# Yelp/nrtsearch

Hardware: AMD Instinct MI355X
Metric: queries/sec, 10M-doc 5-term BM25 top-1000 (higher is better)
Workload: dtype f32

## Files before the change

include/nrtgpu_dev.h:

```cpp
#ifndef NRTGPU_DEV_H
#define NRTGPU_DEV_H
#include "nrtgpu.h"
#ifdef __cplusplus
extern "C" {
#endif
int  nrtgpu_bench_closed_loop(nrtgpu_ctx* ctx, const nrtgpu_seg* const* segs, const int32_t* doc_bases, int32_t n_segs,
                              const nrtgpu_bm25_query* queries, int32_t n_queries, int32_t clients, int32_t duration_ms,
                              double* out4);
int  nrtgpu_debug_hold_coalescers(nrtgpu_ctx* ctx, int32_t hold);
int  nrtgpu_debug_coalescer_pending(nrtgpu_ctx* ctx, int32_t which);
int  nrtgpu_debug_dist_inject(nrtgpu_ctx* ctx, int32_t step, int32_t failed_query);
int64_t nrtgpu_debug_live_segments(nrtgpu_ctx* ctx);
int  nrtgpu_debug_spec_counters(nrtgpu_ctx* ctx, int64_t* out3);
int  nrtgpu_debug_term_lookup(const nrtgpu_seg* seg, int32_t field_id, int64_t term_hash, int32_t* kind, int32_t* shift, int64_t* bytes);
int  nrtgpu_debug_knn_bounds(int32_t sim, int32_t dim, double q_norm2, double q_l1, float q_absmax, double nv_max, double nv_min,
                             float rows_absmax, float score_boost, double m, double s, double* out10);

#define NRTGPU_FLAG_PROFILE (7 << 8)
int  nrtgpu_get_scan_profile(nrtgpu_ctx* ctx, double* out16);
int  nrtgpu_get_maxscore_profile(nrtgpu_ctx* ctx, double* out16);
int64_t nrtgpu_get_maxscore_item_walls(nrtgpu_ctx* ctx, uint64_t* out, int64_t cap_slots, int64_t* n_items);

#ifdef __cplusplus
}
#endif
#endif
```

nrtsearch_amd/_lib.py:

```python
from __future__ import annotations

import ctypes as C
import os

_HERE = os.path.dirname(os.path.abspath(__file__))
LIB_PATH = os.environ.get("NRTGPU_LIB_PATH") or os.path.join(_HERE, "libnrtgpu.so")

NRTGPU_OK = 0
NRTGPU_ERR_INVALID_ARG = -1
NRTGPU_ERR_HIP = -2
NRTGPU_ERR_OOM = -3
NRTGPU_ERR_UNSUPPORTED = -4
NRTGPU_ERR_STATE = -5
NRTGPU_ERR_TIMEOUT = -6
NRTGPU_MAX_K = 1024
NRTGPU_MAX_TERMS = 32
NRTGPU_TILE_DOCS = 1024
NRTGPU_FLAG_NO_PREFETCH = 1
NRTGPU_FLAG_NO_FIXED_POINT = 2
NRTGPU_FLAG_NO_MASK_VARIANT = 4
NRTGPU_FLAG_NO_LIVE_FOLD = 8
NRTGPU_FLAG_NO_PRUNE = 16
NRTGPU_FLAG_PACKED_POSTINGS = 32
NRTGPU_FLAG_BLOCKING_WAIT = 64
# ... 11 lines not shown
    "nrtgpu_search_bm25_coalesced", "nrtgpu_set_coalescing", "nrtgpu_query_supported",
    "nrtgpu_merge_topk_device", "nrtgpu_knn_exact", "nrtgpu_knn_exact_coalesced", "nrtgpu_knn_search", "nrtgpu_rescore_vectors", "nrtgpu_search_hybrid_batch",
    "nrtgpu_int_to_byte4", "nrtgpu_byte4_to_int", "nrtgpu_bm25_idf", "nrtgpu_bm25_avgdl",
    "nrtgpu_bm25_norm_cache", "nrtgpu_slices", "nrtgpu_plan_item_counts", "nrtgpu_fixed_point_scale", "nrtgpu_get_stats", "nrtgpu_reset_stats",
    "nrtgpu_set_slicing",
    "nrtgpu_blend", "nrtgpu_dist_unique_id", "nrtgpu_dist_init", "nrtgpu_dist_search_bm25_batch", "nrtgpu_dist_allgather_merge", "nrtgpu_segment_fork",
    "nrtgpu_search_bm25_batch_device_begin", "nrtgpu_pending_wait", "nrtgpu_set_thread_deadline_ns", "nrtgpu_monotonic_ns", "nrtgpu_last_diagnostics", "nrtgpu_dist_close", "nrtgpu_dist_owned_range", "nrtgpu_dist_search_bm25_batch_mode", "nrtgpu_dist_exchange_merge", "nrtgpu_dist_exchange_merge_checked", "nrtgpu_search_bm25_shard_device_begin", "nrtgpu_note_shard_speculation", "nrtgpu_dist_knn_exact", "nrtgpu_dist_search_hybrid_batch",
    "nrtgpu_knn_exact_relation", "nrtgpu_set_speculation", "nrtgpu_set_shard_share", "nrtgpu_set_thread_slices",
    "nrtgpu_segment_add_byte_vectors", "nrtgpu_knn_exact_bytes", "nrtgpu_knn_search_bytes", "nrtgpu_byte_vector_score",
    "nrtgpu_rescore_byte_vectors", "nrtgpu_search_hybrid_bytes_batch",
]
DEV_SYMBOLS = [
    "nrtgpu_bench_closed_loop", "nrtgpu_debug_hold_coalescers", "nrtgpu_debug_coalescer_pending", "nrtgpu_debug_live_segments",
    "nrtgpu_debug_spec_counters", "nrtgpu_get_scan_profile", "nrtgpu_get_maxscore_profile", "nrtgpu_get_maxscore_item_walls",
    "nrtgpu_debug_dist_inject", "nrtgpu_debug_term_lookup", "nrtgpu_debug_knn_bounds",
]
DEV_LIB_PATH = os.path.join(_HERE, "libnrtgpu_dev.so")


class Config(C.Structure):
    _fields_ = [("device_id", C.c_int32), ("max_batch", C.c_int32), ("target_items", C.c_int32),
                ("collect_timing", C.c_int32), ("flags", C.c_int32), ("host_threads", C.c_int32),
                ("lookup_budget_pct", C.c_int32), ("reserved", C.c_int32)]


class Term(C.Structure):
    _fields_ = [("field_id", C.c_int32), ("cache_slot", C.c_int32), ("term_hash", C.c_int64),
                ("weight", C.c_float), ("occur", C.c_int32)]


# ... 125 lines not shown
    L.nrtgpu_knn_exact_relation.argtypes = [vp, vp, vp, C.c_int32, C.c_int32, C.c_int32, C.c_int32]
    L.nrtgpu_reset_stats.restype = None
    if hasattr(L, "nrtgpu_debug_hold_coalescers"):
        L.nrtgpu_debug_hold_coalescers.argtypes = [vp, C.c_int32]
        L.nrtgpu_debug_live_segments.argtypes = [vp]
        L.nrtgpu_debug_live_segments.restype = C.c_int64
        L.nrtgpu_debug_spec_counters.argtypes = [vp, vp]
        L.nrtgpu_debug_spec_counters.restype = C.c_int
        L.nrtgpu_get_maxscore_item_walls.argtypes = [vp, vp, C.c_int64, C.POINTER(C.c_int64)]
        L.nrtgpu_get_maxscore_item_walls.restype = C.c_int64
        L.nrtgpu_debug_coalescer_pending.argtypes = [vp, C.c_int32]
        L.nrtgpu_debug_dist_inject.argtypes = [vp, C.c_int32, C.c_int32]
        L.nrtgpu_get_scan_profile.argtypes = [vp, vp]
        L.nrtgpu_get_maxscore_profile.argtypes = [vp, vp]
        L.nrtgpu_debug_term_lookup.argtypes = [vp, i32, i64, C.POINTER(i32), C.POINTER(i32), C.POINTER(i64)]
    if hasattr(L, "nrtgpu_debug_knn_bounds"):
        L.nrtgpu_debug_knn_bounds.argtypes = [i32, i32, C.c_double, C.c_double, f32, C.c_double, C.c_double, f32, f32, C.c_double, C.c_double, vp]
    L.nrtgpu_set_slicing.argtypes = [vp, i32, i32, i32]
    L.nrtgpu_blend.argtypes = [i32, vp, vp, vp, vp, i32, i32, i32, i32, C.POINTER(TopDocs)]
    L.nrtgpu_dist_unique_id.argtypes = [vp]
    L.nrtgpu_dist_init.argtypes = [vp, i32, i32, vp]
    L.nrtgpu_dist_search_bm25_batch.argtypes = [vp, vp, vp, i32, C.POINTER(Bm25Query), i32, C.POINTER(TopDocs)]
    L.nrtgpu_dist_allgather_merge.argtypes = [vp, i32, i32, vp, vp, vp, vp, vp, C.POINTER(TopDocs)]
    L.nrtgpu_segment_fork.argtypes = [vp, vp, i32, C.POINTER(vp)]
    L.nrtgpu_search_bm25_batch_device_begin.argtypes = [vp, vp, vp, i32, C.POINTER(Bm25Query), i32, i32, vp, vp, vp, C.c_int64, vp]
    L.nrtgpu_pending_wait.argtypes = [vp]
    L.nrtgpu_set_thread_deadline_ns.argtypes = [C.c_int64]
    L.nrtgpu_set_thread_deadline_ns.restype = None
    L.nrtgpu_monotonic_ns.argtypes = []
    L.nrtgpu_monotonic_ns.restype = C.c_int64
# ... 19 lines not shown
```

nrtsearch_amd/api.py:

```python
from __future__ import annotations

import ctypes as C
import dataclasses
import os
import threading
from typing import Dict, List, Optional, Sequence, Tuple, Union

import numpy as np

from . import _lib
from ._lib import NrtGpuError

INT_MAX = 2**31 - 1
TOTAL_HITS_THRESHOLD = 1000


EXCHANGE_ALLGATHER, EXCHANGE_ALLTOALL = 0, 1
EXCHANGE_NO_SPECULATION = 0x100


@dataclasses.dataclass(frozen=True)
class TermQuery:
    field: int
    term: int
# ... 193 lines not shown
        out = np.zeros(16, dtype=np.float64)
        _lib.check(_lib.load().nrtgpu_get_scan_profile(self._h, out.ctypes.data))
        names = ["prologue_cycles", "rendezvous_wait_cycles", "rendezvous_cycles", "walk_cycles", "epilogue_cycles",
                 "rendezvous", "compactions", "subtiles", "rz_select_cycles", "sparse_subtiles", "rz_keep_cycles",
                 "rz_publish_append_cycles", "candidate_subtiles", "maybe_subtiles", "last_wave_finish_cycles",
                 "first_wave_finish_cycles"]
        return dict(zip(names, out.tolist()))

    def maxscore_profile(self) -> dict:
        out = np.zeros(16, dtype=np.float64)
        _lib.check(_lib.load().nrtgpu_get_maxscore_profile(self._h, out.ctypes.data))
        names = ["windows", "compactions", "chunks", "postings_streamed", "postings_surviving", "docs_evaluated", "lookups",
                 "candidates", "prologue_cycles", "item_cycles", "waves_meeting_cycles", "waves_idle_cycles", "waves_part_prologue_cycles",
                 "waves_walk_cycles", "last_wave_out_cycles", "epilogue_cycles"]
        return dict(zip(names, out.tolist()))

    @staticmethod
    def set_thread_deadline(seconds_from_now: Optional[float]) -> None:
        L = _lib.load()
        L.nrtgpu_set_thread_deadline_ns(0 if seconds_from_now is None else int(L.nrtgpu_monotonic_ns() + seconds_from_now * 1e9))

    @staticmethod
    def last_diagnostics() -> dict:
        d = _lib.Diagnostics()
        _lib.check(_lib.load().nrtgpu_last_diagnostics(C.byref(d)))
        return {n: getattr(d, n) for n, _ in _lib.Diagnostics._fields_ if n != "reserved"}

    def reset_stats(self) -> None:
        _lib.load().nrtgpu_reset_stats(self._h)

# ... 635 lines not shown
    return out, sh[:n].tolist()


def debug_knn_bounds(sim: int, dim: int, q_norm2: float, q_l1: float, q_absmax: float, nv_max: float, nv_min: float,
                     rows_absmax: float, score_boost: float = 1.0, m: float = 0.0, s: float = 0.0) -> dict:
    out = np.zeros(10, dtype=np.float64)
    _lib.check(_lib.load().nrtgpu_debug_knn_bounds(int(sim), int(dim), float(q_norm2), float(q_l1), C.c_float(q_absmax), float(nv_max),
                                                   float(nv_min), C.c_float(rows_absmax), C.c_float(score_boost), float(m), float(s),
                                                   out.ctypes.data))
    names = ("e32", "e16", "result_upper32", "result_upper16", "estimate_lower32", "estimate_lower16", "q_scale", "rows_scale")
    d = {n: float(out[i]) for i, n in enumerate(names)}
    d["q_scale_usable"], d["rows_scale_usable"] = bool(out[8]), bool(out[9])
    return d


def blend(retriever_docs: Sequence[np.ndarray], retriever_scores: Optional[Sequence[np.ndarray]] = None,
          boosts: Optional[Sequence[float]] = None, mode: str = "rrf", k: int = 60, start_hit: int = 0, top_hits: int = 10) -> TopDocs:
    n = len(retriever_docs)
    docs = [np.ascontiguousarray(d, dtype=np.int32) for d in retriever_docs]
    scs = [np.ascontiguousarray(s_, dtype=np.float32) for s_ in retriever_scores] if retriever_scores is not None else None
    dp = (C.c_void_p * max(n, 1))(*[d.ctypes.data for d in docs])
    sp = (C.c_void_p * max(n, 1))(*[s_.ctypes.data for s_ in scs]) if scs is not None else None
    counts = np.asarray([len(d) for d in docs], dtype=np.int32)
    b = np.ascontiguousarray(boosts, dtype=np.float32) if boosts is not None else None
    cap = max(int(top_hits), 1)
    od, os_ = np.zeros(cap, np.int32), np.zeros(cap, np.float32)
    out = _lib.TopDocs()
    out.capacity = cap
    out.docs = od.ctypes.data_as(C.POINTER(C.c_int32))
    out.scores = os_.ctypes.data_as(C.POINTER(C.c_float))
# ... 22 lines not shown
```

nrtsearch_amd/csrc/devtools.cpp:

```cpp
#include "runtime_internal.h"
#include "../../include/nrtgpu_dev.h"

extern "C" int nrtgpu_bench_closed_loop(nrtgpu_ctx* ctx, const nrtgpu_seg* const* segs, const int32_t* doc_bases,
                                        int32_t n_segs, const nrtgpu_bm25_query* queries, int32_t n_queries,
                                        int32_t clients, int32_t duration_ms, double* out4) {
  if (!ctx || !queries || !out4 || n_queries <= 0 || clients <= 0 || duration_ms <= 0)
    return fail(NRTGPU_ERR_INVALID_ARG, "bad closed-loop arguments");
  std::vector<std::vector<float>> lat((size_t)clients);
  std::vector<int> rcs((size_t)clients, 0);
  std::vector<std::string> errs((size_t)clients);
  const auto t_begin = std::chrono::steady_clock::now();
  const auto t_stop = t_begin + std::chrono::milliseconds(duration_ms);
  auto client = [&](int c) {
    int32_t kmax = 1;
    for (int i = 0; i < n_queries; ++i) kmax = std::max(kmax, queries[i].k);
    std::vector<int32_t> docs((size_t)kmax);
    std::vector<float> scores((size_t)kmax);
    size_t i = (size_t)c * 7919u;
    for (;;) {
      const auto t0 = std::chrono::steady_clock::now();
      if (t0 >= t_stop) break;
      nrtgpu_topdocs o{};
      o.capacity = kmax;
      o.docs = docs.data();
// ... 33 lines not shown
  const double e_rel = (double)hostmath::knn_e_rel(), b = (double)score_boost;
  const float e32 = hostmath::knn_bound32(sim, dim, q_norm2, nv_max, b);
  const float e16 = hostmath::knn_bound16(sim, dim, q_norm2, q_l1, 1.0 / (double)q_scale, nv_max, nv_min, 1.0 / (double)rows_scale, b);
  out10[0] = (double)e32;
  out10[1] = (double)e16;
  out10[2] = knn_result_upper(sim, m, (double)e32, e_rel, b);
  out10[3] = knn_result_upper(sim, m, (double)e16, e_rel, b);
  out10[4] = knn_estimate_lower(sim, s, (double)e32, e_rel, b);
  out10[5] = knn_estimate_lower(sim, s, (double)e16, e_rel, b);
  out10[6] = (double)q_scale;
  out10[7] = (double)rows_scale;
  out10[8] = q_ok ? 1.0 : 0.0;
  out10[9] = rows_ok ? 1.0 : 0.0;
  return NRTGPU_OK;
}
```

nrtsearch_amd/csrc/maxscore.hip:

```cpp
#include <hip/hip_runtime.h>
#include <stdint.h>

#include "bm25_common.hiph"

namespace nrtgpu {

constexpr int kMsWinWords = kMsWinDocs / 32;
constexpr int kSl = kMsSlots;
typedef uint32_t u32x2 __attribute__((ext_vector_type(2)));
typedef const NRT_GLOBAL u32x2* gvec2_ptr;

struct alignas(16) WClause {
  uint64_t docids, fnorm;
  uint64_t begin;
  uint32_t count, pad0;
  float    weight;
  int32_t  fx_scale;
  uint32_t flags;
  uint32_t pad;
  uint64_t u_after;
  uint64_t look;
  uint64_t cells, start;
};
static_assert(sizeof(WClause) == 80, "WClause layout");

struct MsSmem {
  uint64_t cand[kMsCandCap];
  uint32_t tab[kTabTerms][kTabEntries];
  float    cache[kLdsCaches][256];
  uint32_t seen[kMsWaves][kMsWinWords];
  WClause  wc[kMsWaves][kMsMaxTerms];
  TopkScratch sc;
  uint64_t theta;
  uint64_t thr;
  uint32_t cnt;
  uint32_t cnt_valid;
  uint32_t rz_flag;
  uint32_t wins_started;
  uint32_t spec_at;
  uint32_t q_wins;
  uint32_t spec_z16;
  uint32_t spec_grow16;
  unsigned long long* spec_slot;
  uint64_t pick;
  uint32_t role[4];
  uint32_t prune_on;
  uint32_t slot_hits[kSliceSlots];
  uint32_t slot_slice[kSliceSlots];
  uint64_t prof[16];
};
static_assert(sizeof(MsSmem) <= 160 * 1024, "the MaxScore workgroup owns one CU's 160 KiB LDS");

// ... 57 lines not shown
__device__ __forceinline__ ms_args_ptr ms_fresh(const MsArgs* p) {
  uint32_t lo = (uint32_t)(uintptr_t)p, hi = (uint32_t)((uintptr_t)p >> 32);
  asm volatile("" : "+v"(lo), "+v"(hi));
  lo = (uint32_t)__builtin_amdgcn_readfirstlane((int)lo);
  hi = (uint32_t)__builtin_amdgcn_readfirstlane((int)hi);
  return (ms_args_ptr)(((uintptr_t)hi << 32) | (uintptr_t)lo);
}

__device__ __noinline__ void ms_compact(__attribute__((address_space(3))) MsSmem* sp, uint32_t k, int fx_E,
                                        unsigned long long* theta_g, const DExchange* xch, uint32_t query) {
  MsSmem& s = *(MsSmem*)sp;
  const uint32_t tid = threadIdx.x;
  const uint32_t cnt_raw = s.cnt;
  const uint32_t cnt0 = cnt_raw > (uint32_t)kMsCandCap ? s.cnt_valid : cnt_raw;
  __syncthreads();
  const bool exchanging = xch && xch->world > 1u;
  uint32_t r = 0;
  if (s.spec_z16 != 0u && !exchanging && __hip_atomic_load(&s.prune_on, __ATOMIC_RELAXED, __HIP_MEMORY_SCOPE_WORKGROUP) != 0u) {
    const float m = (float)k * fminf(1.0f, (float)s.wins_started / (float)max(s.q_wins, 1u));
    const float rr = m + (float)s.spec_z16 * (1.0f / 16.0f) * sqrtf(m) + 2.0f;
    r = rr < (float)k ? (uint32_t)rr : 0u;
  }
  uint64_t guess = 0;
  if (cnt0 > k) {
    const uint32_t k2 = exchanging ? (k + xch->world - 2u) / (xch->world - 1u) : r;
    const uint64_t thr = topk_kth_union<kMsThreads>(s.cand, cnt0, k, &s.sc, [](auto&&) {}, k2);
    const uint32_t q2_hi = s.sc.q2_hi;
    const uint32_t kept = topk_keep_ge<kMsThreads, kMsCandCap>(s.cand, cnt0, thr, &s.sc);
    if (tid == 0) {
      s.cnt = kept;
      if (thr > s.theta) {
        s.theta = thr;
        s.thr = acc_threshold<true>(thr, fx_E);
      }
      atomicMax(theta_g, (unsigned long long)thr);
      s.prof[1] += 1;
    }
    if (!exchanging && r != 0u && q2_hi != 0u) guess = (uint64_t)q2_hi << 32;
    if (xch && tid < 64u) {
      const uint64_t pb = exchange_bound(*xch, query, q2_hi != 0u ? (uint64_t)q2_hi << 32 : 0ull, tid);
      if (tid == 0 && pb > s.theta) {
        s.theta = pb;
        s.thr = acc_threshold<true>(pb, fx_E);
// ... 13 lines not shown
    }
    const uint32_t ws = s.wins_started;
    s.spec_at = ws >= s.q_wins ? 0u : max(ws * s.spec_grow16 / 16u, ws + (uint32_t)kMsWaves);
  }
  __syncthreads();
  if (tid == 0) s.rz_flag = 0;
  __syncthreads();
}

__device__ __forceinline__ bool ms_meet(MsSmem& s, uint32_t k, int fx_E, unsigned long long* theta_g, const DExchange* xch = nullptr,
                                        uint32_t query = 0) {
  __syncthreads();
  if (!__hip_atomic_load(&s.rz_flag, __ATOMIC_RELAXED, __HIP_MEMORY_SCOPE_WORKGROUP)) return false;
  ms_compact((__attribute__((address_space(3))) MsSmem*)&s, k, fx_E, theta_g, xch, query);
  return true;
}

__device__ __forceinline__ bool ms_reserve(MsSmem& s, uint32_t lane, uint32_t mine, uint32_t& pos) {
  const uint32_t incl = scan64_dpp(mine);
  const uint32_t wave_total = (uint32_t)__builtin_amdgcn_readlane((int)incl, 63);
  uint32_t wbase = 0;
  if (lane == 0) {
    wbase = atomicAdd(&s.cnt, wave_total);
    if (wbase + wave_total > (uint32_t)kMsCandCap) {
      if (wbase <= (uint32_t)kMsCandCap) s.cnt_valid = wbase;
      __hip_atomic_store(&s.rz_flag, 1u, __ATOMIC_RELAXED, __HIP_MEMORY_SCOPE_WORKGROUP);
    }
  }
  wbase = (uint32_t)__builtin_amdgcn_readfirstlane((int)wbase);
  pos = wbase + incl - mine;
// ... 115 lines not shown
    const uint32_t mode = item.flags & 3u;
    const uint32_t win_tiles = (uint32_t)kMsWinTiles >> ((item.flags >> 2) & 3u);
    const uint32_t msm = SHAPES ? q.min_should_match : 0u;
    const bool use_max = SHAPES && q.combine_max != 0u;
    const uint32_t sec_mode = TWO ? q.sec_mode : kMsSecNone;
    const float tie_breaker = TWO ? q.tie_breaker : 0.0f;
    auto loosen = [&](uint64_t t) { return (TWO && sec_mode == kMsSecReqOpt) ? max(t - (t >> 21), (uint64_t)2) - (uint64_t)1 : t; };
    unsigned int* const my_prune_g = as_global(ap->q_prune) + item.query;
    const uint64_t after_key = q.has_after ? pack_key(q.after_score, (uint32_t)q.after_doc) : ~0ull;

    {
      const uint32_t n_lds = min(item.n_caches, (uint32_t)kLdsCaches) * 256u;
      const float* const caches = as_global(ap->caches);
      for (uint32_t i = tid; i < n_lds; i += kMsThreads) (&s.cache[0][0])[i] = caches[item.cache_off + i];
    }
    if (tid == 0) {
      const uint64_t theta0 = __hip_atomic_load(my_theta_g, __ATOMIC_RELAXED, __HIP_MEMORY_SCOPE_AGENT);
      s.theta = theta0;
      s.thr = acc_threshold<true>(theta0, fx_E);
      s.cnt = 0;
      s.cnt_valid = 0;
      s.rz_flag = 0;
      if (!helper) {
        const unsigned long long now0 = (unsigned long long)wall_clock64();
        __hip_atomic_store(hp.item_t0 + my_item, now0, __ATOMIC_RELAXED, __HIP_MEMORY_SCOPE_AGENT);
        if (my_item == 0u) __hip_atomic_store(hp.t_start, now0, __ATOMIC_RELAXED, __HIP_MEMORY_SCOPE_AGENT);
      }
      s.prune_on = mode == kMsModePrune ? 1u : 0u;
      const bool spec = hp.spec_g != nullptr && hp.spec_z16 != 0u;
      s.wins_started = 0;
      s.q_wins = spec ? as_global(ap->q_wins)[item.query] : 0u;
      s.spec_z16 = spec ? hp.spec_z16 : 0u;
      s.spec_slot = spec ? as_global(hp.spec_g) + item.query : nullptr;
      s.spec_at = spec ? max(hp.spec_sched & 255u, 1u) : 0u;
      s.spec_grow16 = max((hp.spec_sched >> 8) & 255u, 17u);
      for (int i = 0; i < kSliceSlots; ++i) s.slot_hits[i] = s.slot_slice[i] = 0u;
      for (int i = 0; i < 16; ++i) s.prof[i] = 0;
    }
    const uint64_t t_item0 = PROF ? __builtin_readcyclecounter() : 0ull;
    const uint64_t wall0 = PROF ? wall_clock64() : 0ull;
    uint64_t tc_meet = 0, tc_part = 0, tc_walk = 0;
    __syncthreads();
    if (xch && tid < 64u) {
      const uint64_t pb = exchange_bound(*xch, item.query, 0ull, tid);
      if (tid == 0 && pb > s.theta) {
        s.theta = pb;
        s.thr = acc_threshold<true>(pb, fx_E);
      }
    }
    for (uint32_t slot = 0; slot < item.n_tabs; ++slot) {
// ... 130 lines not shown
        w.start = mt.start;
        wcl[lane] = w;
      }
      const uint32_t req_mask = TWO ? (uint32_t)__builtin_amdgcn_ballot_w64(lane < n_terms && (mt.tab_slot & kTabSlotRequired) != 0u) : 0u;
      const uint32_t first_req = req_mask != 0u ? (uint32_t)__builtin_ctz(req_mask) : 0xFFu;
      if (PROF) tc_part += __builtin_readcyclecounter() - t_part0;

      for (;;) {
        const uint64_t t_win0 = PROF ? __builtin_readcyclecounter() : 0ull;
        const uint32_t ta = (part.tile_begin & ~(win_tiles - 1u)) + (g - win_base) * win_tiles;
        const uint32_t t0 = max(ta, part.tile_begin);
        const uint32_t t1 = min(ta + win_tiles, part.tile_end);
        const uint32_t doc_lo = t0 * (uint32_t)kTileDocs;
        const uint32_t doc_span = min(t1 * (uint32_t)kTileDocs, part.max_doc) - doc_lo;
        if (PROF) pc_wins += 1;
        if (lane == 0) {
          const uint32_t ws = atomicAdd(&s.wins_started, 1u) + 1u, at = s.spec_at;
          if (at != 0u && ws >= at) __hip_atomic_store(&s.rz_flag, 1u, __ATOMIC_RELAXED, __HIP_MEMORY_SCOPE_WORKGROUP);
        }
        uint32_t g_new = 0;
        if (lane == 0) g_new = (uint32_t)kMsWaves + __hip_atomic_fetch_add(win_next_g, 1u, __ATOMIC_RELAXED, __HIP_MEMORY_SCOPE_AGENT);
        uint64_t theta_other = 0, thr_other = 0;
        if (multi_item) {
          theta_other = __hip_atomic_load(my_theta_g, __ATOMIC_RELAXED, __HIP_MEMORY_SCOPE_AGENT);
          thr_other = acc_threshold<true>(theta_other, fx_E);
          if (mode == kMsModeCount && lane == 0 && __hip_atomic_load(my_prune_g, __ATOMIC_RELAXED, __HIP_MEMORY_SCOPE_AGENT) != 0u)
            __hip_atomic_store(&s.prune_on, 1u, __ATOMIC_RELAXED, __HIP_MEMORY_SCOPE_WORKGROUP);
        }
        uint32_t my_lo = 0, my_hi = 0;
        if (lane < n_terms) {
          my_lo = my_cells[t0 >> my_shift];
          my_hi = my_cells[((t1 - 1u) >> my_shift) + 1u];
        }
// ... 473 lines not shown
    if (tid == 0) {
      as_global(ape->item_counts)[out_slot] = n;
      if (helper)
        as_global(hpe.help_query)[out_slot - hpe.slot_base] = item.query + 1u;
      uint32_t hits = 0;
      for (int i = 0; i < kSliceSlots; ++i) {
        const uint32_t h = s.slot_hits[i];
        hits += h;
        if (h != 0u && q.gte_floor != 0xFFFFFFFFu) atomicAdd(as_global(ape->slice_sum) + q.slice_base + s.slot_slice[i], h);
      }
      const bool pruned = s.prune_on != 0u && (s.theta != 0ull || __hip_atomic_load(my_theta_g, __ATOMIC_RELAXED, __HIP_MEMORY_SCOPE_AGENT) != 0ull);
      as_global(ape->item_hits)[out_slot] = (uint64_t)hits + (pruned ? kHitsPrunedUnit : 0ull);
      if (PROF && ape->item_prof) {
  #ifndef NRT_MS_PHASE_CLOCKS
        s.prof[5] = hits;
  #endif
        const uint64_t t_end = __builtin_readcyclecounter();
        s.prof[9] = t_end - t_item0;
        s.prof[15] = t_end - t_epi0;
        for (int i = 0; i < 16; ++i) as_global(ape->item_prof)[(size_t)out_slot * 16 + i] = s.prof[i];
        if (hpe.walls) {
          unsigned long long* const wr = as_global(hpe.walls) + (size_t)out_slot * 8;
          wr[0] = wall0;
          wr[1] = wall_clock64();
          wr[2] = (unsigned long long)my_item | ((unsigned long long)item.flags << 32);
          wr[3] = s.prof[0];
          wr[4] = wall_entry;
          wr[5] = ((unsigned long long)((uint32_t)__builtin_amdgcn_s_getreg((31 << 11) | 20) & 15u) << 8) |
                  (unsigned long long)(((uint32_t)__builtin_amdgcn_s_getreg((31 << 11) | 4) >> 8) & 255u);
          wr[6] = (unsigned long long)round | ((unsigned long long)item.query << 32);
// ... 81 lines not shown
  const uint32_t n_cells = ((max_doc - 1u) >> shift) + 1u;
  uint32_t* const out = (uint32_t*)(look_base + t_look[t]);
  const uint32_t stride = gridDim.x * blockDim.x;
  for (uint32_t i = blockIdx.x * blockDim.x + threadIdx.x; i <= n_cells; i += stride) {
    const uint64_t bound = (uint64_t)i << shift;
    uint32_t lo = 0, hi = n;
    while (lo < hi) {
      const uint32_t mid = (lo + hi) >> 1;
      if ((uint64_t)dd[mid] < bound) lo = mid + 1u;
      else hi = mid;
    }
    out[i] = lo;
  }
}

void launch_bm25_maxscore(hipStream_t stream, bool profile, bool packed, int shapes, const MsArgs& args, const MsArgs* args_d) {
  const uint32_t n_items = args.help.n_own;
  if (n_items == 0) return;
  const uint32_t grid = args.help.persistent ? std::min(n_items + args.help.n_help, std::max(args.help.n_cus, 1u)) : n_items + args.help.n_help;
#define NRT_MS_LAUNCH(P, K, S) hipLaunchKernelGGL((bm25_maxscore_kernel<P, K, S>), dim3(grid), dim3(kMsThreads), 0, stream, args_d)
#define NRT_MS_LAUNCH_S(P, K)          \
  do {                                 \
    if (shapes == 2) NRT_MS_LAUNCH(P, K, 2);      \
    else if (shapes == 1) NRT_MS_LAUNCH(P, K, 1); \
    else NRT_MS_LAUNCH(P, K, 0);                  \
  } while (0)
#ifdef NRTGPU_DEV
  if (profile) {
    if (packed) NRT_MS_LAUNCH_S(true, true);
    else NRT_MS_LAUNCH_S(true, false);
// ... 42 lines not shown
```

nrtsearch_amd/csrc/runtime.cpp:

```cpp
#include "runtime_internal.h"

namespace nrtgpu {
namespace rt {
thread_local std::string g_last_error;
thread_local int64_t g_deadline_ns = 0;
thread_local nrtgpu_diagnostics g_diag{};
thread_local std::vector<int32_t> g_thread_slices;
int64_t monotonic_ns() {
  timespec ts;
  clock_gettime(CLOCK_MONOTONIC, &ts);
  return (int64_t)ts.tv_sec * 1000000000ll + (int64_t)ts.tv_nsec;
}

int fail(int code, const char* fmt, ...) {
  char buf[1024];
  va_list ap;
  va_start(ap, fmt);
  vsnprintf(buf, sizeof(buf), fmt, ap);
  va_end(ap);
  g_last_error = buf;
  return code;
}


// ... 272 lines not shown
  if (!ctx || !out) return fail(NRTGPU_ERR_INVALID_ARG, "NULL argument");
  std::lock_guard<std::mutex> lk(ctx->stats_mu);
  *out = ctx->stats;
  out->spec_queries = ctx->spec_queries.load(std::memory_order_relaxed);
  out->spec_reruns = ctx->spec_reruns.load(std::memory_order_relaxed);
  out->spec_disabled = ctx->spec_off.load(std::memory_order_relaxed);
  out->spec_scattered = ctx->spec_scattered.load(std::memory_order_relaxed);
  return NRTGPU_OK;
}
extern "C" void nrtgpu_reset_stats(nrtgpu_ctx* ctx) {
  if (!ctx) return;
  std::lock_guard<std::mutex> lk(ctx->stats_mu);
  ctx->stats = nrtgpu_stats{};
  for (double& p : ctx->prof) p = 0;
  for (double& p : ctx->ms_prof) p = 0;
}
#ifdef NRTGPU_DEV
extern "C" int nrtgpu_get_scan_profile(nrtgpu_ctx* ctx, double* out16) {
  if (!ctx || !out16) return fail(NRTGPU_ERR_INVALID_ARG, "NULL argument");
  std::lock_guard<std::mutex> lk(ctx->stats_mu);
  for (int i = 0; i < 16; ++i) out16[i] = ctx->prof[i];
  return NRTGPU_OK;
}

extern "C" int nrtgpu_get_maxscore_profile(nrtgpu_ctx* ctx, double* out16) {
  if (!ctx || !out16) return fail(NRTGPU_ERR_INVALID_ARG, "NULL argument");
  std::lock_guard<std::mutex> lk(ctx->stats_mu);
  for (int i = 0; i < 16; ++i) out16[i] = ctx->ms_prof[i];
  return NRTGPU_OK;
}
// ... 77 lines not shown
```

nrtsearch_amd/csrc/runtime_internal.h:

```cpp
#pragma once
#include <hip/hip_runtime.h>
#include <fcntl.h>
#include <stdarg.h>
#include <stdio.h>
#include <string.h>
#include <sys/mman.h>
#include <unistd.h>

#include <algorithm>
#include <atomic>
#include <cerrno>
#include <climits>
#include <cmath>
#include <chrono>
#include <condition_variable>
#include <deque>
#include <functional>
#include <map>
#include <memory>
#include <mutex>
#include <optional>
#include <shared_mutex>
#include <string>
#include <thread>
// ... 1 lines not shown
#include <vector>

#include "../../include/nrtgpu.h"
#ifdef NRTGPU_DEV
#include "../../include/nrtgpu_dev.h"
#endif
#include "host_math.h"
#include "plan.h"

namespace nrtgpu {
void launch_bm25_scan(hipStream_t stream, bool fixed_point, bool pipelined, bool packed, int ablation, uint32_t n_items, const DItem* items,
                      const DPart* parts, const DTerm* terms, const DQuery* queries, const float* caches, unsigned long long* theta_g,
                      unsigned long long* quant_g, const DExchange* xch, uint32_t* slice_sum, uint64_t* item_keys, uint32_t* item_counts,
                      uint64_t* item_hits, uint32_t k_stride, uint64_t* item_prof);
void launch_bm25_maxscore(hipStream_t stream, bool profile, bool packed, int shapes, const MsArgs& args, const MsArgs* args_d);
void launch_term_frontier(hipStream_t stream, const uint32_t* fnorm, const uint64_t* t_start, const uint32_t* t_count,
                          const uint64_t* t_look, const uint32_t* t_meta, const void* look_base, uint32_t n_terms, DTermAux* out);
void launch_term_bits(hipStream_t stream, const uint32_t* docids, const uint64_t* t_start, const uint32_t* t_count, const uint64_t* t_look,
                      const uint32_t* which, uint32_t n_which, uint32_t max_count, void* look_base);
void launch_term_cells(hipStream_t stream, const uint32_t* docids, const uint64_t* t_start, const uint32_t* t_count, const uint64_t* t_look,
                       const uint32_t* t_meta, const uint32_t* which, uint32_t n_which, uint32_t max_cells, uint32_t max_doc, void* look_base);
void launch_expand_terms(hipStream_t stream, const DQExpand* qx, const DQTerm* qterms, const uint32_t* out_begin, uint32_t n_queries,
                         uint32_t n_leaves, DTerm* out);
void launch_slice_relation(hipStream_t stream, const uint32_t* slice_sum, const DQuery* queries, uint32_t n_slices, uint64_t* out_hits,
                           uint32_t n);
void launch_patch_hits(hipStream_t stream, const uint64_t* lower, uint64_t* hits, uint32_t n);
void launch_merge_topk(hipStream_t stream, uint32_t n_queries, const uint64_t* in_keys, const uint32_t* in_counts,
                       const uint64_t* in_hits, const uint32_t* list_idx, const uint32_t* q_base,
                       const uint32_t* q_nlists, uint32_t k_stride_in, const uint32_t* q_k, uint64_t* out_keys,
                       uint32_t* out_counts, uint64_t* out_hits, uint32_t k_stride_out, const uint32_t* help_query = nullptr,
// ... 383 lines not shown
  int device = 0;
  int n_cus = 0;
  std::mutex mu;
  std::condition_variable cv;
  std::vector<std::unique_ptr<Slot>> slots;
  hipEvent_t last_turn = nullptr;
  hipEvent_t last_knn_turn = nullptr;
  std::mutex gpu_mu;
  std::mutex stats_mu;
  nrtgpu_stats stats{};
  std::atomic<int> knn_sketch_skip[4] = {};
  double prof[16] = {0};
  std::vector<uint64_t> last_walls;
  int64_t last_walls_items = 0;
  double ms_prof[16] = {0};
  std::mutex co_mu;
  std::condition_variable co_cv;
  std::vector<struct CoRequest*> co_pending;
  struct CoRequest* co_leader = nullptr;
  int co_inflight = 0;
  int co_inflight_queries = 0;
  int co_last_batch = 0;
  int32_t co_linger_us = 150;
  std::atomic<int64_t> spec_queries{0}, spec_reruns{0};
  std::atomic<int> spec_off{0};
  std::atomic<int> spec_scattered{0};
  std::atomic<uint64_t> spec_epoch{1};
  std::atomic<int> spec_z16{5 * 16};
  std::atomic<int64_t> shard_docs{0}, index_docs{0};
  std::atomic<int64_t> live_segments{0};
// ... 233 lines not shown
```

nrtsearch_amd/csrc/search.cpp:

```cpp
#include "runtime_internal.h"


static uint32_t spec_margin16(const nrtgpu_ctx* ctx) { return (uint32_t)std::max(ctx->spec_z16.load(std::memory_order_relaxed), 0); }
static void spec_sync_epoch(const nrtgpu_ctx* ctx, LeafSetCache* lsc) {
  const uint64_t e = ctx->spec_epoch.load(std::memory_order_relaxed);
  if (lsc->spec_epoch.exchange(e, std::memory_order_relaxed) != e) {
    lsc->spec_queries.store(0, std::memory_order_relaxed);
    lsc->spec_reruns.store(0, std::memory_order_relaxed);
    lsc->spec_calls.store(0, std::memory_order_relaxed);
    lsc->spec_calls_rerun.store(0, std::memory_order_relaxed);
    lsc->spec_scattered.store(0, std::memory_order_relaxed);
    lsc->spec_off.store(0, std::memory_order_relaxed);
  }
}
static bool speculating(nrtgpu_ctx* ctx, const nrtgpu_seg* const* segs, int32_t n_segs) {
  if (!ctx || spec_margin16(ctx) == 0u || !segs || n_segs <= 0) return false;
  for (int32_t i = 0; i < n_segs; ++i)
    if (!segs[i]) return false;
  std::shared_ptr<LeafSetCache> lsc = leaf_set_cache(ctx, segs, n_segs);
  spec_sync_epoch(ctx, lsc.get());
  return lsc->spec_off.load(std::memory_order_relaxed) == 0;
}
static void note_speculation_of(nrtgpu_ctx* ctx, LeafSetCache* lsc, int64_t n_queries, int64_t n_rerun) {
  spec_sync_epoch(ctx, lsc);
// ... 156 lines not shown
    help.alpha16 = (uint32_t)std::max(env_help_alpha, 0);
    static const int env_spare = (int)dev_env_int("NRTGPU_MS_SPARE_CUS", 8);
    help.n_cus = (uint32_t)std::max(ctx->n_cus - std::max(env_spare, 0), 1);
    if (small) help.n_cus = (uint32_t)std::max(env_spare, 1);
    help.persistent = ms_persistent() ? 1u : 0u;
  }
  help.n_own = (uint32_t)hp.n_ms_items;
  help.n_help = (uint32_t)n_help;
  help.slot_base = (uint32_t)n_items;
  static const bool env_help_greedy = dev_env_int("NRTGPU_MS_HELP_GREEDY", 0) != 0;
  help.min_rem = (uint32_t)std::min(std::max(env_help_min, 1), 0xFFFF) | (env_help_greedy ? 1u << 16 : 0u);
  help.walls = profile ? (unsigned long long*)(wb + o_walls) : nullptr;
  help.spec_g = spec ? (unsigned long long*)(wb + o_spec) : nullptr;
  help.spec_z16 = spec ? spec_z16 : 0u;
  {
    static const int env_first = (int)dev_env_int("NRTGPU_MS_SPEC_FIRST", 2 * kMsWaves);
    static const int env_grow = (int)dev_env_int("NRTGPU_MS_SPEC_GROW", 32);
    help.spec_sched = (uint32_t)std::min(std::max(env_first, 1), 255) | ((uint32_t)std::min(std::max(env_grow, 17), 255) << 8);
  }
  MsArgs ms_args{};
  ms_args.items = (const DItem*)(db + o_items);
  ms_args.parts = (const DPart*)(db + o_parts);
  ms_args.terms = (const DTerm*)(wb + o_terms);
  ms_args.queries = (const DQuery*)(db + o_queries);
  ms_args.caches = (const float*)(db + o_caches);
  ms_args.theta_g = (unsigned long long*)(db + o_theta);
  ms_args.slice_sum = (uint32_t*)(wb + o_ssum);
  ms_args.q_prune = (uint32_t*)(wb + o_qprune);
  ms_args.xch = use_xch ? (const DExchange*)(db + o_xch) : nullptr;
  ms_args.item_keys = (uint64_t*)(wb + o_ikeys);
  ms_args.item_counts = (uint32_t*)(wb + o_icnt);
  ms_args.item_hits = (uint64_t*)(wb + o_ihits);
  ms_args.item_prof = profile ? (uint64_t*)(wb + o_prof) : nullptr;
// ... 175 lines not shown
      for (int qi = q0; qi < q1; ++qi)
        unpack_topdocs(keys + (size_t)qi * hp.k_stride, cnts[qi], hits[qi] & ~kHitsSpecInvalid, queries[qi].k, hp.q_lower[(size_t)qi], cnts[qi], &out[qi]);
    });
  }
  if (rerun)
    for (int qi = 0; qi < n_queries; ++qi)
      if (hits[qi] & kHitsSpecInvalid) rerun->push_back(qi);
  if (call_trace)
    fprintf(stderr, "[nrtgpu call] %d queries: plan %.3f ms, upload + kernels %.3f, results to host %.3f, unpack %.3f\n", n_queries, plan_ms,
            tc1 - tc0, tc2 - tc1, now_ms() - tc2);
  if (run.prof && run.n_items) {
    std::vector<uint64_t> hp_prof(run.n_slots * 16);
    HIP_TRY(hipMemcpy(hp_prof.data(), run.prof, hp_prof.size() * 8, hipMemcpyDeviceToHost));
    std::lock_guard<std::mutex> lk(ctx->stats_mu);
    for (size_t i = 0; i < run.n_slots; ++i)
      for (int j = 0; j < 16; ++j) ((i < run.n_ms_items || i >= run.n_items) ? ctx->ms_prof : ctx->prof)[j] += (double)hp_prof[i * 16 + j];
    if (run.walls) {
      std::vector<uint64_t> w(run.n_slots * 8);
      (void)hipMemcpy(w.data(), run.walls, w.size() * 8, hipMemcpyDeviceToHost);
      ctx->last_walls.swap(w);
      ctx->last_walls_items = (int64_t)run.n_ms_items;
    }
  }
  account(ctx, slot, hp, n_queries, plan_ms, t0, queue_ms);
  return NRTGPU_OK;
}

static int search_batch_spec(nrtgpu_ctx* ctx, const nrtgpu_seg* const* segs, const int32_t* doc_bases, int32_t n_segs,
                             const nrtgpu_bm25_query* queries, int32_t n_queries, nrtgpu_topdocs* out,
                             const std::function<void(const std::vector<int32_t>&)>* after_first) {
  std::vector<int32_t> rerun;
// ... 769 lines not shown
```

Before: 517,900.

## Replace block-wide speculative meeting with single-wave kth threshold estimate

By default, a wave that reaches the speculation schedule point now claims a busy flag and runs a single-wave kth-largest estimate over the LDS candidate buffer. It raises theta from that estimate directly, instead of setting the rendezvous flag that forces all waves into a block-wide compaction meeting. The aim is to cut the synchronisation stalls of the meetings while still tightening the pruning threshold early. The old meeting path stays available behind an environment variable. Candidate slots are now zero-filled so the wave can read them safely, and profiling counters for meetings and estimates are added. The cost is the estimating wave pausing its own work and a possibly less accurate threshold.

```diff
diff --git a/include/nrtgpu_dev.h b/include/nrtgpu_dev.h
--- a/include/nrtgpu_dev.h
+++ b/include/nrtgpu_dev.h
@@ -19,6 +19,8 @@
 #define NRTGPU_FLAG_PROFILE (7 << 8)
 int  nrtgpu_get_scan_profile(nrtgpu_ctx* ctx, double* out16);
 int  nrtgpu_get_maxscore_profile(nrtgpu_ctx* ctx, double* out16);
+int  nrtgpu_debug_maxscore_meetings(nrtgpu_ctx* ctx, int64_t* out4);
+int  nrtgpu_debug_wave_kth(const uint64_t* keys, int32_t n, int32_t r, uint64_t* out);
 int64_t nrtgpu_get_maxscore_item_walls(nrtgpu_ctx* ctx, uint64_t* out, int64_t cap_slots, int64_t* n_items);
 
 #ifdef __cplusplus
diff --git a/nrtsearch_amd/_lib.py b/nrtsearch_amd/_lib.py
--- a/nrtsearch_amd/_lib.py
+++ b/nrtsearch_amd/_lib.py
@@ -49,6 +49,7 @@
     "nrtgpu_bench_closed_loop", "nrtgpu_debug_hold_coalescers", "nrtgpu_debug_coalescer_pending", "nrtgpu_debug_live_segments",
     "nrtgpu_debug_spec_counters", "nrtgpu_get_scan_profile", "nrtgpu_get_maxscore_profile", "nrtgpu_get_maxscore_item_walls",
     "nrtgpu_debug_dist_inject", "nrtgpu_debug_term_lookup", "nrtgpu_debug_knn_bounds",
+    "nrtgpu_debug_maxscore_meetings", "nrtgpu_debug_wave_kth",
 ]
 DEV_LIB_PATH = os.path.join(_HERE, "libnrtgpu_dev.so")
 
@@ -204,6 +205,9 @@
         L.nrtgpu_get_scan_profile.argtypes = [vp, vp]
         L.nrtgpu_get_maxscore_profile.argtypes = [vp, vp]
         L.nrtgpu_debug_term_lookup.argtypes = [vp, i32, i64, C.POINTER(i32), C.POINTER(i32), C.POINTER(i64)]
+    if hasattr(L, "nrtgpu_debug_maxscore_meetings"):
+        L.nrtgpu_debug_maxscore_meetings.argtypes = [vp, vp]
+        L.nrtgpu_debug_wave_kth.argtypes = [vp, i32, i32, vp]
     if hasattr(L, "nrtgpu_debug_knn_bounds"):
         L.nrtgpu_debug_knn_bounds.argtypes = [i32, i32, C.c_double, C.c_double, f32, C.c_double, C.c_double, f32, f32, C.c_double, C.c_double, vp]
     L.nrtgpu_set_slicing.argtypes = [vp, i32, i32, i32]
diff --git a/nrtsearch_amd/api.py b/nrtsearch_amd/api.py
--- a/nrtsearch_amd/api.py
+++ b/nrtsearch_amd/api.py
@@ -231,6 +231,11 @@
                  "candidates", "prologue_cycles", "item_cycles", "waves_meeting_cycles", "waves_idle_cycles", "waves_part_prologue_cycles",
                  "waves_walk_cycles", "last_wave_out_cycles", "epilogue_cycles"]
         return dict(zip(names, out.tolist()))
+
+    def maxscore_meetings(self) -> dict:
+        out = np.zeros(4, dtype=np.int64)
+        _lib.check(_lib.load().nrtgpu_debug_maxscore_meetings(self._h, out.ctypes.data))
+        return dict(zip(["meetings", "overflow_meetings", "compactions", "wave_estimates"], (int(x) for x in out)))
 
     @staticmethod
     def set_thread_deadline(seconds_from_now: Optional[float]) -> None:
@@ -896,6 +901,13 @@
     return d
 
 
+def debug_wave_kth(keys: np.ndarray, r: int) -> int:
+    keys = np.ascontiguousarray(keys, dtype=np.uint64)
+    out = np.zeros(1, dtype=np.uint64)
+    _lib.check(_lib.load().nrtgpu_debug_wave_kth(keys.ctypes.data, len(keys), int(r), out.ctypes.data))
+    return int(out[0])
+
+
 def blend(retriever_docs: Sequence[np.ndarray], retriever_scores: Optional[Sequence[np.ndarray]] = None,
           boosts: Optional[Sequence[float]] = None, mode: str = "rrf", k: int = 60, start_hit: int = 0, top_hits: int = 10) -> TopDocs:
     n = len(retriever_docs)
diff --git a/nrtsearch_amd/csrc/devtools.cpp b/nrtsearch_amd/csrc/devtools.cpp
--- a/nrtsearch_amd/csrc/devtools.cpp
+++ b/nrtsearch_amd/csrc/devtools.cpp
@@ -71,3 +71,25 @@
   out10[9] = rows_ok ? 1.0 : 0.0;
   return NRTGPU_OK;
 }
+
+extern "C" int nrtgpu_debug_maxscore_meetings(nrtgpu_ctx* ctx, int64_t* out4) {
+  if (!ctx || !out4) return fail(NRTGPU_ERR_INVALID_ARG, "NULL argument");
+  std::lock_guard<std::mutex> lk(ctx->stats_mu);
+  for (int i = 0; i < 4; ++i) out4[i] = ctx->ms_meetings[i];
+  return NRTGPU_OK;
+}
+
+extern "C" int nrtgpu_debug_wave_kth(const uint64_t* keys, int32_t n, int32_t r, uint64_t* out) {
+  if (!keys || !out || n < 1 || n > kMsCandCap || r < 1 || r > n) return fail(NRTGPU_ERR_INVALID_ARG, "bad wave_kth arguments (1 <= r <= n <= %d)", kMsCandCap);
+  uint64_t* d = nullptr;
+  if (hipMalloc((void**)&d, ((size_t)n + 1) * sizeof(uint64_t)) != hipSuccess) return fail(NRTGPU_ERR_OOM, "hipMalloc");
+  hipError_t e = hipMemcpy(d, keys, (size_t)n * sizeof(uint64_t), hipMemcpyHostToDevice);
+  if (e == hipSuccess) {
+    launch_debug_wave_kth(nullptr, d, (uint32_t)n, (uint32_t)r, d + n);
+    e = hipGetLastError();
+  }
+  if (e == hipSuccess) e = hipMemcpy(out, d + n, sizeof(uint64_t), hipMemcpyDeviceToHost);
+  (void)hipFree(d);
+  if (e != hipSuccess) return fail(NRTGPU_ERR_HIP, "wave_kth: %s", hipGetErrorString(e));
+  return NRTGPU_OK;
+}
diff --git a/nrtsearch_amd/csrc/maxscore.hip b/nrtsearch_amd/csrc/maxscore.hip
--- a/nrtsearch_amd/csrc/maxscore.hip
+++ b/nrtsearch_amd/csrc/maxscore.hip
@@ -36,6 +36,9 @@
   uint32_t cnt;
   uint32_t cnt_valid;
   uint32_t rz_flag;
+  uint32_t spec_busy;
+  uint32_t spec_meet;
+  uint32_t n_meet, n_over, n_est;
   uint32_t wins_started;
   uint32_t spec_at;
   uint32_t q_wins;
@@ -123,6 +126,10 @@
   const uint32_t cnt_raw = s.cnt;
   const uint32_t cnt0 = cnt_raw > (uint32_t)kMsCandCap ? s.cnt_valid : cnt_raw;
   __syncthreads();
+  if (tid == 0) {
+    s.n_meet += 1u;
+    if (cnt_raw > (uint32_t)kMsCandCap) s.n_over += 1u;
+  }
   const bool exchanging = xch && xch->world > 1u;
   uint32_t r = 0;
   if (s.spec_z16 != 0u && !exchanging && __hip_atomic_load(&s.prune_on, __ATOMIC_RELAXED, __HIP_MEMORY_SCOPE_WORKGROUP) != 0u) {
@@ -136,6 +143,7 @@
     const uint64_t thr = topk_kth_union<kMsThreads>(s.cand, cnt0, k, &s.sc, [](auto&&) {}, k2);
     const uint32_t q2_hi = s.sc.q2_hi;
     const uint32_t kept = topk_keep_ge<kMsThreads, kMsCandCap>(s.cand, cnt0, thr, &s.sc);
+    for (uint32_t i = kept + tid; i < (uint32_t)kMsCandCap; i += kMsThreads) s.cand[i] = 0ull;
     if (tid == 0) {
       s.cnt = kept;
       if (thr > s.theta) {
@@ -179,6 +187,38 @@
   if (!__hip_atomic_load(&s.rz_flag, __ATOMIC_RELAXED, __HIP_MEMORY_SCOPE_WORKGROUP)) return false;
   ms_compact((__attribute__((address_space(3))) MsSmem*)&s, k, fx_E, theta_g, xch, query);
   return true;
+}
+
+__device__ __noinline__ void ms_estimate(__attribute__((address_space(3))) MsSmem* sp, uint32_t k, int fx_E,
+                                         unsigned long long* theta_g, const DExchange* xch) {
+  MsSmem& s = *(MsSmem*)sp;
+  const uint32_t lane = threadIdx.x & 63u;
+  const uint32_t ws = (uint32_t)__builtin_amdgcn_readfirstlane((int)__hip_atomic_load(&s.wins_started, __ATOMIC_RELAXED, __HIP_MEMORY_SCOPE_WORKGROUP));
+  const uint32_t at = (uint32_t)__builtin_amdgcn_readfirstlane((int)__hip_atomic_load(&s.spec_at, __ATOMIC_RELAXED, __HIP_MEMORY_SCOPE_WORKGROUP));
+  const uint32_t n = (uint32_t)__builtin_amdgcn_readfirstlane((int)__hip_atomic_load(&s.cnt, __ATOMIC_RELAXED, __HIP_MEMORY_SCOPE_WORKGROUP));
+  if (at != 0u && ws >= at && n <= (uint32_t)kMsCandCap) {
+    const bool exchanging = xch && xch->world > 1u;
+    uint32_t r = 0;
+    if (s.spec_z16 != 0u && !exchanging && __hip_atomic_load(&s.prune_on, __ATOMIC_RELAXED, __HIP_MEMORY_SCOPE_WORKGROUP) != 0u) {
+      const float m = (float)k * fminf(1.0f, (float)ws / (float)max(s.q_wins, 1u));
+      const float rr = m + (float)s.spec_z16 * (1.0f / 16.0f) * sqrtf(m) + 2.0f;
+      r = rr < (float)k ? (uint32_t)rr : 0u;
+    }
+    uint64_t guess = 0;
+    if (r != 0u && n > r) guess = topk_kth_wave(s.cand, n, r, &s.sc);
+    if (lane == 0u) {
+      if (guess > s.theta) {
+        __hip_atomic_store(&s.theta, guess, __ATOMIC_RELAXED, __HIP_MEMORY_SCOPE_WORKGROUP);
+        __hip_atomic_store(&s.thr, acc_threshold<true>(guess, fx_E), __ATOMIC_RELAXED, __HIP_MEMORY_SCOPE_WORKGROUP);
+        atomicMax(theta_g, (unsigned long long)guess);
+        atomicMax(s.spec_slot, (unsigned long long)guess);
+      }
+      s.spec_at = ws >= s.q_wins ? 0u : max(ws * s.spec_grow16 / 16u, ws + (uint32_t)kMsWaves);
+      s.n_est += 1u;
+    }
+  }
+  wave_lds_phase();
+  if (lane == 0u) __hip_atomic_store(&s.spec_busy, 0u, __ATOMIC_RELEASE, __HIP_MEMORY_SCOPE_WORKGROUP);
 }
 
 __device__ __forceinline__ bool ms_reserve(MsSmem& s, uint32_t lane, uint32_t mine, uint32_t& pos) {
@@ -324,6 +364,7 @@
       const float* const caches = as_global(ap->caches);
       for (uint32_t i = tid; i < n_lds; i += kMsThreads) (&s.cache[0][0])[i] = caches[item.cache_off + i];
     }
+    for (uint32_t i = tid; i < (uint32_t)kMsCandCap; i += kMsThreads) s.cand[i] = 0ull;
     if (tid == 0) {
       const uint64_t theta0 = __hip_atomic_load(my_theta_g, __ATOMIC_RELAXED, __HIP_MEMORY_SCOPE_AGENT);
       s.theta = theta0;
@@ -331,6 +372,8 @@
       s.cnt = 0;
       s.cnt_valid = 0;
       s.rz_flag = 0;
+      s.spec_busy = 0;
+      s.n_meet = s.n_over = s.n_est = 0;
       if (!helper) {
         const unsigned long long now0 = (unsigned long long)wall_clock64();
         __hip_atomic_store(hp.item_t0 + my_item, now0, __ATOMIC_RELAXED, __HIP_MEMORY_SCOPE_AGENT);
@@ -344,6 +387,7 @@
       s.spec_slot = spec ? as_global(hp.spec_g) + item.query : nullptr;
       s.spec_at = spec ? max(hp.spec_sched & 255u, 1u) : 0u;
       s.spec_grow16 = max((hp.spec_sched >> 8) & 255u, 17u);
+      s.spec_meet = (hp.spec_sched >> 16) & 1u;
       for (int i = 0; i < kSliceSlots; ++i) s.slot_hits[i] = s.slot_slice[i] = 0u;
       for (int i = 0; i < 16; ++i) s.prof[i] = 0;
     }
@@ -504,9 +548,17 @@
         const uint32_t doc_lo = t0 * (uint32_t)kTileDocs;
         const uint32_t doc_span = min(t1 * (uint32_t)kTileDocs, part.max_doc) - doc_lo;
         if (PROF) pc_wins += 1;
-        if (lane == 0) {
-          const uint32_t ws = atomicAdd(&s.wins_started, 1u) + 1u, at = s.spec_at;
-          if (at != 0u && ws >= at) __hip_atomic_store(&s.rz_flag, 1u, __ATOMIC_RELAXED, __HIP_MEMORY_SCOPE_WORKGROUP);
+        {
+          uint32_t est = 0;
+          if (lane == 0) {
+            const uint32_t ws = atomicAdd(&s.wins_started, 1u) + 1u, at = s.spec_at;
+            if (at != 0u && ws >= at) {
+              if (s.spec_meet != 0u) __hip_atomic_store(&s.rz_flag, 1u, __ATOMIC_RELAXED, __HIP_MEMORY_SCOPE_WORKGROUP);
+              else est = atomicCAS(&s.spec_busy, 0u, 1u) == 0u ? 1u : 0u;
+            }
+          }
+          if (__builtin_amdgcn_readfirstlane((int)est) != 0)
+            ms_estimate((__attribute__((address_space(3))) MsSmem*)&s, k, fx_E, my_theta_g, xch);
         }
         uint32_t g_new = 0;
         if (lane == 0) g_new = (uint32_t)kMsWaves + __hip_atomic_fetch_add(win_next_g, 1u, __ATOMIC_RELAXED, __HIP_MEMORY_SCOPE_AGENT);
@@ -1010,6 +1062,7 @@
       if (PROF && ape->item_prof) {
   #ifndef NRT_MS_PHASE_CLOCKS
         s.prof[5] = hits;
+        s.prof[1] = (s.prof[1] & 0xFFFFull) | ((uint64_t)min(s.n_meet, 0xFFFFu) << 16) | ((uint64_t)min(s.n_over, 0xFFFFu) << 32) | ((uint64_t)min(s.n_est, 0xFFFFu) << 48);
   #endif
         const uint64_t t_end = __builtin_readcyclecounter();
         s.prof[9] = t_end - t_item0;
@@ -1121,6 +1174,22 @@
   }
 }
 
+#ifdef NRTGPU_DEV
+__global__ __launch_bounds__(64)
+void debug_wave_kth_kernel(const uint64_t* __restrict__ keys, uint32_t n, uint32_t r, uint64_t* __restrict__ out) {
+  __shared__ uint64_t cand[kMsCandCap];
+  __shared__ TopkScratch sc;
+  for (uint32_t i = threadIdx.x; i < n; i += 64u) cand[i] = keys[i];
+  wave_lds_phase();
+  const uint64_t kth = topk_kth_wave(cand, n, r, &sc);
+  if (threadIdx.x == 0) *out = kth;
+}
+
+void launch_debug_wave_kth(hipStream_t stream, const uint64_t* keys, uint32_t n, uint32_t r, uint64_t* out) {
+  hipLaunchKernelGGL(debug_wave_kth_kernel, dim3(1), dim3(64), 0, stream, keys, n, r, out);
+}
+#endif
+
 void launch_bm25_maxscore(hipStream_t stream, bool profile, bool packed, int shapes, const MsArgs& args, const MsArgs* args_d) {
   const uint32_t n_items = args.help.n_own;
   if (n_items == 0) return;
diff --git a/nrtsearch_amd/csrc/runtime.cpp b/nrtsearch_amd/csrc/runtime.cpp
--- a/nrtsearch_amd/csrc/runtime.cpp
+++ b/nrtsearch_amd/csrc/runtime.cpp
@@ -310,6 +310,7 @@
   ctx->stats = nrtgpu_stats{};
   for (double& p : ctx->prof) p = 0;
   for (double& p : ctx->ms_prof) p = 0;
+  for (int64_t& p : ctx->ms_meetings) p = 0;
 }
 #ifdef NRTGPU_DEV
 extern "C" int nrtgpu_get_scan_profile(nrtgpu_ctx* ctx, double* out16) {
diff --git a/nrtsearch_amd/csrc/runtime_internal.h b/nrtsearch_amd/csrc/runtime_internal.h
--- a/nrtsearch_amd/csrc/runtime_internal.h
+++ b/nrtsearch_amd/csrc/runtime_internal.h
@@ -39,6 +39,9 @@
                       unsigned long long* quant_g, const DExchange* xch, uint32_t* slice_sum, uint64_t* item_keys, uint32_t* item_counts,
                       uint64_t* item_hits, uint32_t k_stride, uint64_t* item_prof);
 void launch_bm25_maxscore(hipStream_t stream, bool profile, bool packed, int shapes, const MsArgs& args, const MsArgs* args_d);
+#ifdef NRTGPU_DEV
+void launch_debug_wave_kth(hipStream_t stream, const uint64_t* keys, uint32_t n, uint32_t r, uint64_t* out);
+#endif
 void launch_term_frontier(hipStream_t stream, const uint32_t* fnorm, const uint64_t* t_start, const uint32_t* t_count,
                           const uint64_t* t_look, const uint32_t* t_meta, const void* look_base, uint32_t n_terms, DTermAux* out);
 void launch_term_bits(hipStream_t stream, const uint32_t* docids, const uint64_t* t_start, const uint32_t* t_count, const uint64_t* t_look,
@@ -452,6 +455,7 @@
   std::vector<uint64_t> last_walls;
   int64_t last_walls_items = 0;
   double ms_prof[16] = {0};
+  int64_t ms_meetings[4] = {0};
   std::mutex co_mu;
   std::condition_variable co_cv;
   std::vector<struct CoRequest*> co_pending;
diff --git a/nrtsearch_amd/csrc/search.cpp b/nrtsearch_amd/csrc/search.cpp
--- a/nrtsearch_amd/csrc/search.cpp
+++ b/nrtsearch_amd/csrc/search.cpp
@@ -194,9 +194,10 @@
   help.spec_g = spec ? (unsigned long long*)(wb + o_spec) : nullptr;
   help.spec_z16 = spec ? spec_z16 : 0u;
   {
-    static const int env_first = (int)dev_env_int("NRTGPU_MS_SPEC_FIRST", 2 * kMsWaves);
-    static const int env_grow = (int)dev_env_int("NRTGPU_MS_SPEC_GROW", 32);
-    help.spec_sched = (uint32_t)std::min(std::max(env_first, 1), 255) | ((uint32_t)std::min(std::max(env_grow, 17), 255) << 8);
+    const int env_first = (int)dev_env_int("NRTGPU_MS_SPEC_FIRST", 2 * kMsWaves);
+    const int env_grow = (int)dev_env_int("NRTGPU_MS_SPEC_GROW", 32);
+    const bool env_meet = dev_env_int("NRTGPU_MS_SPEC_MEET", 0) != 0;
+    help.spec_sched = (uint32_t)std::min(std::max(env_first, 1), 255) | ((uint32_t)std::min(std::max(env_grow, 17), 255) << 8) | (env_meet ? 1u << 16 : 0u);
   }
   MsArgs ms_args{};
   ms_args.items = (const DItem*)(db + o_items);
@@ -402,7 +403,19 @@
     HIP_TRY(hipMemcpy(hp_prof.data(), run.prof, hp_prof.size() * 8, hipMemcpyDeviceToHost));
     std::lock_guard<std::mutex> lk(ctx->stats_mu);
     for (size_t i = 0; i < run.n_slots; ++i)
-      for (int j = 0; j < 16; ++j) ((i < run.n_ms_items || i >= run.n_items) ? ctx->ms_prof : ctx->prof)[j] += (double)hp_prof[i * 16 + j];
+      if (i < run.n_ms_items || i >= run.n_items) {
+#ifndef NRT_MS_PHASE_CLOCKS
+        const uint64_t packed = hp_prof[i * 16 + 1];
+        hp_prof[i * 16 + 1] = packed & 0xFFFFull;
+        ctx->ms_meetings[0] += (int64_t)((packed >> 16) & 0xFFFFull);
+        ctx->ms_meetings[1] += (int64_t)((packed >> 32) & 0xFFFFull);
+        ctx->ms_meetings[2] += (int64_t)(packed & 0xFFFFull);
+        ctx->ms_meetings[3] += (int64_t)(packed >> 48);
+#endif
+        for (int j = 0; j < 16; ++j) ctx->ms_prof[j] += (double)hp_prof[i * 16 + j];
+      } else {
+        for (int j = 0; j < 16; ++j) ctx->prof[j] += (double)hp_prof[i * 16 + j];
+      }
     if (run.walls) {
       std::vector<uint64_t> w(run.n_slots * 8);
       (void)hipMemcpy(w.data(), run.walls, w.size() * 8, hipMemcpyDeviceToHost);
```

Measured after the change: 523,100, median of 6. 1.0% higher.
